# raider99k/UNINA-YOLO-DLA

Measured on NVIDIA B200. Metric: images/sec @640x640 (forward + DFL decode + NMS), higher is better.
Workload: dtype bf16

## Files before the change

unina-yolo-dla_b200/csrc/stem_fused.cu:

```cuda
#include <type_traits>

#include "camera.cuh"
#include "stem_v2.cuh"

#include "common.cuh"

namespace uyd {

struct StemArgs {
  const void *in;
  __nv_bfloat16 *out;
  const uint32_t *wfrag;
  const float *bias;
  int n, ih, iw, oh, ow, out_pitch, u8;
  int pw;
  CamFrames f;
};

namespace stemv2 {
__device__ __forceinline__ void mma1688_tf32(float (&d)[4], const uint4 &a, uint32_t b0, uint32_t b1) {
  asm volatile(
      "mma.sync.aligned.m16n8k8.row.col.f32.tf32.tf32.f32 {%0,%1,%2,%3}, {%4,%5,%6,%7}, {%8,%9}, {%0,%1,%2,%3};"
      : "+f"(d[0]), "+f"(d[1]), "+f"(d[2]), "+f"(d[3])
      : "r"(a.x), "r"(a.y), "r"(a.z), "r"(a.w), "r"(b0), "r"(b1));
}
__device__ __forceinline__ void mma16816v(float (&d)[4], const uint4 &a, uint32_t b0, uint32_t b1) {
  asm volatile(
      "mma.sync.aligned.m16n8k16.row.col.f32.bf16.bf16.f32 {%0,%1,%2,%3}, {%4,%5,%6,%7}, {%8,%9}, {%0,%1,%2,%3};"
      : "+f"(d[0]), "+f"(d[1]), "+f"(d[2]), "+f"(d[3])
      : "r"(a.x), "r"(a.y), "r"(a.z), "r"(a.w), "r"(b0), "r"(b1));
}
__device__ __forceinline__ uint32_t movmatrix_trans(uint32_t v) {
  uint32_t r;
  asm volatile("movmatrix.sync.aligned.m8n8.trans.b16 %0, %1;" : "=r"(r) : "r"(v));
  return r;
}

template <typename TIn, bool PW, bool PERSIST>
__global__ void __launch_bounds__(stemv2::kThreads, PERSIST ? 2 : 3) stem_v2_kernel(StemArgs a) {
  pdl_trigger();
  extern __shared__ __align__(16) unsigned char smem[];
  unsigned char *patch = smem;
  unsigned char *l0s = smem + kPatchBytes;
  unsigned char *w1s = smem + kPatchBytes + kL0Bytes;

  const int tid = threadIdx.x, warp = tid >> 5, lane = tid & 31, g = lane >> 2, t = lane & 3;
  uint4 w1r[PERSIST ? 18 : 1];
  if (PERSIST) {
#pragma unroll
    for (int i = 0; i < (PERSIST ? 18 : 0); ++i) w1r[i] = __ldg(reinterpret_cast<const uint4 *>(a.wfrag + kW0Words) + i * 32 + lane);
  }
  const int tiles_x = (a.ow + kTW - 1) / kTW, tiles_y = (a.oh + kTH - 1) / kTH;
  const int total_tiles = PERSIST ? tiles_x * tiles_y * a.n : 1;
  for (int tile = PERSIST ? (int)blockIdx.x : 0; tile < total_tiles; tile += PERSIST ? (int)gridDim.x : 1) {
  int ox0, oy0, n;
  if (PERSIST) {
    const int per = tiles_x * tiles_y, r = tile % per;
    n = tile / per; oy0 = (r / tiles_x) * kTH; ox0 = (r % tiles_x) * kTW;
  } else {
    ox0 = blockIdx.x * kTW; oy0 = blockIdx.y * kTH; n = blockIdx.z;
  }
  const int ix0 = 4 * ox0 - 4, iy0 = 4 * oy0 - 3;

  constexpr int kW1Vec = kW1Words / 4, kWIters = (kW1Vec + kThreads - 1) / kThreads;
  const uint4 *w1g = reinterpret_cast<const uint4 *>(a.wfrag + kW0Words);
  uint4 wv[kWIters];
#pragma unroll
  for (int it = 0; it < kWIters; ++it) {
    const int i = tid + it * kThreads;
    wv[it] = (!PERSIST && i < kW1Vec) ? __ldg(w1g + i) : make_uint4(0u, 0u, 0u, 0u);
  }
  constexpr int kVecPerRow = kInW / 4, kRowLanes = 15;
  static_assert(2 * kRowLanes <= kInH && 3 * kRowLanes >= kInH && kRowLanes * kVecPerRow <= kThreads, "patch load map");
  constexpr bool kLetterbox = std::is_same<TIn, CamLetterboxIn>::value;
  constexpr bool kCam = std::is_same<TIn, CamIn>::value || kLetterbox;
  const TIn *img = reinterpret_cast<const TIn *>(a.in) + (kCam ? 0ll : (long long)n * 3 * a.ih * a.iw);
  asm volatile("" : "+l"(img));
  const int pj = tid % kVecPerRow, prl = tid / kVecPerRow;
  const int ix = ix0 + 4 * pj;
  const bool col_ok = prl < kRowLanes && ix >= 0 && ix + 3 < a.iw;
  const unsigned plane = (unsigned)(a.ih * a.iw);
  bool ok[3];
  unsigned off[3];
#pragma unroll
  for (int k = 0; k < 3; ++k) {
    const int r = prl + kRowLanes * k, iy = iy0 + r;
    ok[k] = col_ok && r < kInH && (unsigned)iy < (unsigned)a.ih;
    off[k] = (unsigned)(iy * a.iw + ix);
  }
  uint4 pv[3][3];
  if constexpr (kCam) {
    const uint8_t *frame = reinterpret_cast<const uint8_t *>(a.in) + (long long)n * a.f.frame_stride;
    const uint8_t *uvp = a.f.uv ? a.f.uv + (long long)n * a.f.uv_frame_stride : nullptr;
    const CamNorm nm = cam_norm(a.f);
    CamLetterbox lb;
    if constexpr (kLetterbox) lb = cam_letterbox(a, a.f);
#pragma unroll
    for (int k = 0; k < 3; ++k) {
      float px[4][3];
#pragma unroll
      for (int j = 0; j < 4; ++j) px[j][0] = px[j][1] = px[j][2] = 0.f;
      if (ok[k]) {
        if constexpr (kLetterbox) cam_letterbox4(lb, a.f, nm, frame, iy0 + prl + kRowLanes * k, ix, px);
        else cam_row4(a, a.f, nm, frame, uvp, iy0 + prl + kRowLanes * k, ix, px);
      }
#pragma unroll
      for (int c = 0; c < 3; ++c)
        pv[c][k] = make_uint4(__float_as_uint(px[0][c]), __float_as_uint(px[1][c]), __float_as_uint(px[2][c]), __float_as_uint(px[3][c]));
    }
  } else {
#pragma unroll
  for (int c = 0; c < 3; ++c)
#pragma unroll
    for (int k = 0; k < 3; ++k) {
      pv[c][k] = make_uint4(0u, 0u, 0u, 0u);
      if (ok[k]) {
        const TIn *src = img + (off[k] + c * plane);
        if (sizeof(TIn) == 4) pv[c][k] = __ldg(reinterpret_cast<const uint4 *>(src));
        else pv[c][k].x = __ldg(reinterpret_cast<const unsigned int *>(src));
      }
    }
  }
#pragma unroll
  for (int it = 0; it < kWIters; ++it) {
    const int i = tid + it * kThreads;
    if (!PERSIST && i < kW1Vec) reinterpret_cast<uint4 *>(w1s)[i] = wv[it];
  }
#pragma unroll
  for (int k = 0; k < 3; ++k) {
    const int r = prl + kRowLanes * k;
    if (prl < kRowLanes && r < kInH) {
      unsigned char *dst = patch + (patch_line(0, r) * kInW + 4 * pj) * 4;
#pragma unroll
      for (int c = 0; c < 3; ++c) {
        const uint4 v = pv[c][k];
        uint4 o;
        if (sizeof(TIn) == 4 || kCam) {
          o = ok[k] ? make_uint4(v.x + 0x1000u, v.y + 0x1000u, v.z + 0x1000u, v.w + 0x1000u) : v;
        } else {
          auto cv = [&](uint32_t b) { return ok[k] ? __float_as_uint(div255((float)b)) + 0x1000u : 0u; };
          o = make_uint4(cv(v.x & 0xffu), cv((v.x >> 8) & 0xffu), cv((v.x >> 16) & 0xffu), cv(v.x >> 24));
        }
        *reinterpret_cast<uint4 *>(dst + c * kChanLines * kInW * 4) = o;
      }
    }
  }
  __syncthreads();

  {
    const uint4 *w0g = reinterpret_cast<const uint4 *>(a.wfrag);
    uint4 af[5];
#pragma unroll
    for (int s = 0; s < 5; ++s) af[s] = __ldg(w0g + s * 32 + lane);
    const float b_lo = __ldg(a.bias + g), b_hi = __ldg(a.bias + g + 8);
    const unsigned char *pb[5];
#pragma unroll
    for (int s = 0; s < 5; ++s)
      pb[s] = patch + 64 * warp + 8 * g + 8 * (t & 1) + 4 * ((t >> 1) ? l0_k_off(s, 2) : l0_k_off(s, 0));
    unsigned char *sb = l0s + (8 * warp + 2 * t) * kL0Pitch + 4 * g;
    auto groups = [&](int i0, auto cnt) {
      constexpr int NG = decltype(cnt)::value;
      float acc[NG][4];
#pragma unroll
      for (int j = 0; j < NG; ++j) { acc[j][0] = acc[j][1] = b_lo; acc[j][2] = acc[j][3] = b_hi; }
#pragma unroll
      for (int s = 0; s < 5; ++s) {
        uint2 v[NG];
#pragma unroll
        for (int j = 0; j < NG; ++j) v[j] = ld64(pb[s] + 512 * (i0 + j));
#pragma unroll
        for (int j = 0; j < NG; ++j) mma1688_tf32(acc[j], af[s], v[j].x, v[j].y);
      }
#pragma unroll
      for (int j = 0; j < NG; ++j) {
        st32(sb + 64 * kL0Pitch * (i0 + j), relu_pack_bf16(acc[j][0], acc[j][2]));
        st32(sb + 64 * kL0Pitch * (i0 + j) + kL0Pitch, relu_pack_bf16(acc[j][1], acc[j][3]));
      }
    };
    static_assert(kGroups == 73, "nine groups per warp and one more for warp 0");
    groups(0, std::integral_constant<int, 3>{});
    groups(3, std::integral_constant<int, 3>{});
    groups(6, std::integral_constant<int, 3>{});
    if (warp == 0) groups(9, std::integral_constant<int, 1>{});
  }
  __syncthreads();
  if (oy0 == 0 || ox0 == 0) {
    if (oy0 == 0)
      for (int i = tid; i < kL0P * 8; i += kThreads) st32(l0s + (i >> 3) * kL0Pitch + 4 * (i & 7), 0u);
    if (ox0 == 0 && tid < kL0H * 8) st32(l0s + (tid >> 3) * kL0P * kL0Pitch + 4 * (tid & 7), 0u);
    __syncthreads();
  }

  {
    float acc[2][2][4];
#pragma unroll
    for (int mt = 0; mt < 2; ++mt) {
      const float2 bz = __ldg(reinterpret_cast<const float2 *>(a.bias + 16 + 4 * g + 2 * mt));
#pragma unroll
      for (int xg = 0; xg < 2; ++xg) { acc[xg][mt][0] = acc[xg][mt][1] = bz.x; acc[xg][mt][2] = acc[xg][mt][3] = bz.y; }
    }
    const unsigned char *bb = l0s + l1_b_off(warp, 0, g, t, 0);
    const uint4 *wf = reinterpret_cast<const uint4 *>(w1s) + lane;
#pragma unroll
    for (int tap = 0; tap < 9; ++tap) {
      const uint4 a0 = PERSIST ? w1r[PERSIST ? tap * 2 : 0] : wf[(tap * 2 + 0) * 32], a1 = PERSIST ? w1r[PERSIST ? tap * 2 + 1 : 0] : wf[(tap * 2 + 1) * 32];
#pragma unroll
      for (int xg = 0; xg < 2; ++xg) {
        const uint2 b = ld64(bb + ((tap / 3) * kL0P + 16 * xg + tap % 3) * kL0Pitch);
        mma16816v(acc[xg][0], a0, b.x, b.y);
        mma16816v(acc[xg][1], a1, b.x, b.y);
      }
    }
    const int oy = oy0 + warp;
    __nv_bfloat16 *orow = a.out + ((long long)n * a.oh + oy) * a.ow * a.out_pitch;
    if (!PW) {
#pragma unroll
      for (int xg = 0; xg < 2; ++xg)
#pragma unroll
        for (int h = 0; h < 2; ++h) {
          const int px = ox0 + 8 * xg + 2 * t + h;
          if (oy < a.oh && px < a.ow)
            *reinterpret_cast<uint2 *>(orow + (long long)px * a.out_pitch + 4 * g) =
                make_uint2(relu_pack_bf16(acc[xg][0][h], acc[xg][0][2 + h]), relu_pack_bf16(acc[xg][1][h], acc[xg][1][2 + h]));
        }
    } else {
      const uint4 *w2 = reinterpret_cast<const uint4 *>(a.wfrag + kW0Words + kW1Words) + lane;
      const uint4 p0 = __ldg(w2), p1 = __ldg(w2 + 32);
      const float2 bz = __ldg(reinterpret_cast<const float2 *>(a.bias + 48 + 2 * g));
#pragma unroll
      for (int xg = 0; xg < 2; ++xg) {
        float acc2[4] = {bz.x, bz.x, bz.y, bz.y};
        uint32_t bq[2][2];
#pragma unroll
        for (int mt = 0; mt < 2; ++mt)
#pragma unroll
          for (int hh = 0; hh < 2; ++hh) bq[mt][hh] = movmatrix_trans(relu_pack_bf16(acc[xg][mt][2 * hh], acc[xg][mt][2 * hh + 1]));
        mma16816v(acc2, p0, bq[0][0], bq[0][1]);
        mma16816v(acc2, p1, bq[1][0], bq[1][1]);
#pragma unroll
        for (int h = 0; h < 2; ++h) {
          const int px = ox0 + 8 * xg + 2 * t + h;
          if (oy < a.oh && px < a.ow)
            *reinterpret_cast<uint32_t *>(orow + (long long)px * a.out_pitch + 2 * g) = relu_pack_bf16(acc2[h], acc2[2 + h]);
        }
      }
    }
  }
  }
}
}
bool stem_fused_supported(int c0, int c1, int ih, int iw, int out_pitch, int out_coff) {
  return c0 == 16 && c1 == 32 && ih % 4 == 0 && iw % 4 == 0 && out_pitch % 8 == 0 && out_coff % 8 == 0;
}

void stem_fused_pack(const float *w0, const float *b0, const float *w1, const float *b1, const float *w2, const float *b2,
                     std::vector<uint32_t> &frags, std::vector<float> &bias) {
  frags.clear();
  bias.assign(64, 0.f);
  for (int i = 0; i < 16; ++i) bias[i] = b0[i];
  for (int i = 0; i < 32; ++i) bias[16 + i] = b1[i];
  for (int i = 0; i < 16 && b2; ++i) bias[48 + i] = b2[i];
  stemv2::pack(w0, w1, w2, frags);
}

static int stem_v2_launch(const StemArgs &a0, cudaStream_t s) {
  StemArgs a = a0;
  static const bool persist = [] { const char *v = getenv("UYD_STEM_PERSIST"); return !(v && *v == '0'); }();
  const int sms = current_sm_count();
  UYD_REQUIRE(sms > 0, UYD_E_NOGPU, "stem: no current CUDA device");
  const int tiles = ceil_div(a.ow, stemv2::kTW) * ceil_div(a.oh, stemv2::kTH) * a.n;
  const size_t smem = stemv2::kSmemBytes;
  auto go = [&](auto kern, bool pers) -> int {
    if (int e = smem_optin(kern, stemv2::kSmemBytes)) return e;
    if (pers) kern<<<tiles < 2 * sms ? tiles : 2 * sms, stemv2::kThreads, smem, s>>>(a);
    else kern<<<dim3(ceil_div(a.ow, stemv2::kTW), ceil_div(a.oh, stemv2::kTH), a.n), stemv2::kThreads, smem, s>>>(a);
    return (int)cudaGetLastError();
  };
  const bool pers = persist && tiles >= 8 * sms;
  using namespace stemv2;
  if (a.f.cam == UYD_CAM_BGRA_LETTERBOX) {
    if (a.pw) return pers ? go(stem_v2_kernel<CamLetterboxIn, true, true>, true) : go(stem_v2_kernel<CamLetterboxIn, true, false>, false);
    return pers ? go(stem_v2_kernel<CamLetterboxIn, false, true>, true) : go(stem_v2_kernel<CamLetterboxIn, false, false>, false);
  }
  if (a.f.cam) {
    if (a.pw) return pers ? go(stem_v2_kernel<CamIn, true, true>, true) : go(stem_v2_kernel<CamIn, true, false>, false);
    return pers ? go(stem_v2_kernel<CamIn, false, true>, true) : go(stem_v2_kernel<CamIn, false, false>, false);
  }
  if (a.u8) {
    if (a.pw) return pers ? go(stem_v2_kernel<uint8_t, true, true>, true) : go(stem_v2_kernel<uint8_t, true, false>, false);
    return pers ? go(stem_v2_kernel<uint8_t, false, true>, true) : go(stem_v2_kernel<uint8_t, false, false>, false);
  }
  if (a.pw) return pers ? go(stem_v2_kernel<float, true, true>, true) : go(stem_v2_kernel<float, true, false>, false);
  return pers ? go(stem_v2_kernel<float, false, true>, true) : go(stem_v2_kernel<float, false, false>, false);
}

int stem_fused_launch(const StemArgs &a, cudaStream_t s) { return stem_v2_launch(a, s); }

}
```

unina-yolo-dla_b200/csrc/stem_v2.cuh:

```cuda
#pragma once
#include "c3k_flat.cuh"

namespace uyd {
namespace stemv2 {
using c3kf::host_f2bf;
using c3kf::ld64;
using c3kf::relu_pack_bf16;
using c3kf::st32;

constexpr int kTH = 8, kTW = 16;
constexpr int kL0H = 2 * kTH + 1, kL0P = 2 * kTW + 2;
constexpr int kGroups = (16 * kL0P + 2 * kTW + 1 + 7) / 8;
constexpr int kL0Px = kGroups * 8;
constexpr int kInH = 2 * kL0H + 1, kInW = 2 * kL0P;
constexpr int kOddLine = 20, kChanLines = 38;
constexpr int kL0Pitch = 48;
constexpr int kPatchBytes = 3 * kChanLines * kInW * 4;
constexpr int kL0Bytes = kL0Px * kL0Pitch;
constexpr int kW0Words = 5 * 128, kW1Words = 9 * 2 * 128, kW2Words = 2 * 128;
constexpr int kSmemBytes = kPatchBytes + kL0Bytes + kW1Words * 4;
constexpr int kThreads = 256;
constexpr int kFragWords = kW0Words + kW1Words + kW2Words;

C3K_HD int patch_line(int c, int r) { return c * kChanLines + ((r & 1) ? kOddLine + (r >> 1) : (r >> 1)); }

C3K_HD int l0_k_off(int s, int t) {
  int c = 2 * s + (t >> 1);
  if (c > 8) c = 8;
  const int ky = c % 3;
  return (patch_line(c / 3, ky & 1) + (ky >> 1)) * kInW + 2 * (t & 1);
}
inline float l0_weight(const float *w0, int s, int k, int n) {
  const int t = k & 3, combo = 2 * s + (t >> 1), slot = 2 * (t & 1) + (k >> 2), kx = slot - 1;
  if (combo > 8 || kx < 0) return 0.f;
  return w0[((n * 3 + combo / 3) * 3 + combo % 3) * 3 + kx];
}
C3K_HD void l0_store(unsigned char *l0s, int q, int g, float lo_ch, float hi_ch) { st32(l0s + q * kL0Pitch + 4 * g, relu_pack_bf16(lo_ch, hi_ch)); }

C3K_HD int l1_k_chan(int kk) { return 2 * ((kk & 7) >> 1) + (kk >> 3) + 8 * (kk & 1); }
C3K_HD int l1_b_off(int row, int xg, int g, int t, int tap) {
  return ((2 * row + tap / 3) * kL0P + 2 * (8 * xg + g) + tap % 3) * kL0Pitch + 8 * t;
}
C3K_HD int l1_chan(int mt, int r) { return 4 * (r & 7) + 2 * mt + (r >> 3); }

C3K_HD int pw_chan(int r) { return 2 * (r & 7) + (r >> 3); }

inline uint32_t f32_bits(float f) { uint32_t u; memcpy(&u, &f, 4); return u; }
inline float bits_f32(uint32_t u) { float f; memcpy(&f, &u, 4); return f; }
inline float bf16_round(float f) { return bits_f32((uint32_t)host_f2bf(f) << 16); }

C3K_HD float div255(float x) {
#if defined(__CUDA_ARCH__)
  const float r = 1.0f / 255.0f;
  const float q = __fmul_rn(x, r);
  return __fmaf_rn(__fmaf_rn(-q, 255.0f, x), r, q);
#else
  return x / 255.0f;
#endif
}

inline void pack(const float *w0, const float *w1, const float *w2 , std::vector<uint32_t> &out) {
  for (int s = 0; s < 5; ++s)
    for (int lane = 0; lane < 32; ++lane) {
      const int g = lane >> 2, t = lane & 3;
      auto w = [&](int row, int k) { return f32_bits(bf16_round(l0_weight(w0, s, k, row))); };
      out.push_back(w(g, t)); out.push_back(w(g + 8, t)); out.push_back(w(g, t + 4)); out.push_back(w(g + 8, t + 4));
    }
  for (int tap = 0; tap < 9; ++tap)
    for (int mt = 0; mt < 2; ++mt)
      for (int lane = 0; lane < 32; ++lane) {
        const int g = lane >> 2, t = lane & 3;
        auto w = [&](int row, int kk) {
          auto one = [&](int k1) { return (uint32_t)host_f2bf(w1[(l1_chan(mt, row) * 16 + l1_k_chan(k1)) * 9 + tap]); };
          return one(kk) | (one(kk + 1) << 16);
        };
        out.push_back(w(g, 2 * t)); out.push_back(w(g + 8, 2 * t)); out.push_back(w(g, 2 * t + 8)); out.push_back(w(g + 8, 2 * t + 8));
      }
  for (int ks = 0; ks < 2; ++ks)
    for (int lane = 0; lane < 32; ++lane) {
      const int g = lane >> 2, t = lane & 3;
      auto w = [&](int row, int kk) {
        auto one = [&](int k1) { return w2 ? (uint32_t)host_f2bf(w2[pw_chan(row) * 32 + l1_chan(ks, k1)]) : 0u; };
        return one(kk) | (one(kk + 1) << 16);
      };
      out.push_back(w(g, 2 * t)); out.push_back(w(g + 8, 2 * t)); out.push_back(w(g, 2 * t + 8)); out.push_back(w(g + 8, 2 * t + 8));
    }
}

}
}
```

Before: 32890.

## Load fp32 stem input patches with double-buffered TMA in persistent kernel

Adds a TMA path for fp32 non-camera input in the persistent stem kernel. A 4D tensor map splits even and odd rows, and thread 0 prefetches the next tile's 3-channel patch into a second shared-memory buffer, tracked by mbarriers. This replaces per-thread global loads and shared stores. Out-of-bounds zero fill replaces the explicit edge masking, and the tf32 rounding offset is now applied at fragment load time. The cost is a larger shared-memory footprint and a host-side tensor map encode on every launch.

```diff
diff --git a/unina-yolo-dla_b200/csrc/stem_fused.cu b/unina-yolo-dla_b200/csrc/stem_fused.cu
--- a/unina-yolo-dla_b200/csrc/stem_fused.cu
+++ b/unina-yolo-dla_b200/csrc/stem_fused.cu
@@ -4,6 +4,7 @@
 #include "stem_v2.cuh"
 
 #include "common.cuh"
+#include "tc_ptx.cuh"
 
 namespace uyd {
 
@@ -36,13 +37,31 @@
   return r;
 }
 
+struct TmaF32 {};
+template <typename TIn>
+using StemMap = typename std::conditional<std::is_same<TIn, TmaF32>::value, CUtensorMap, char>::type;
+
+__device__ __forceinline__ void stem_tma_patch(const CUtensorMap *tm, unsigned char *buf, uint32_t bar, int ox0, int oy0, int n) {
+  mbar_expect_tx(bar, 6 * kTmaRows * kInW * 4);
+#pragma unroll
+  for (int c = 0; c < 3; ++c)
+#pragma unroll
+    for (int odd = 0; odd < 2; ++odd) {
+      const int line0 = patch_line(c, odd, true), lead = tma_lead(c, odd);
+      tma_load_4d(smem_u32(buf + (line0 - lead) * kInW * 4), tm, bar, 4 * ox0 - 4, 1 - odd, 2 * oy0 - 2 + odd - lead, 3 * n + c);
+    }
+}
+
 template <typename TIn, bool PW, bool PERSIST>
-__global__ void __launch_bounds__(stemv2::kThreads, PERSIST ? 2 : 3) stem_v2_kernel(StemArgs a) {
+__global__ void __launch_bounds__(stemv2::kThreads, PERSIST ? 2 : 3) stem_v2_kernel(StemArgs a, const __grid_constant__ StemMap<TIn> tm) {
+  constexpr bool kTma = std::is_same<TIn, TmaF32>::value;
+  static_assert(!kTma || PERSIST, "the TMA patch pipeline walks tiles");
   pdl_trigger();
-  extern __shared__ __align__(16) unsigned char smem[];
+  extern __shared__ __align__(128) unsigned char smem[];
   unsigned char *patch = smem;
-  unsigned char *l0s = smem + kPatchBytes;
+  unsigned char *l0s = smem + (kTma ? 2 * kTmaBufBytes : kPatchBytes);
   unsigned char *w1s = smem + kPatchBytes + kL0Bytes;
+  const uint32_t full_bar = smem_u32(smem + 2 * kTmaBufBytes + kL0Bytes);
 
   const int tid = threadIdx.x, warp = tid >> 5, lane = tid & 31, g = lane >> 2, t = lane & 3;
   uint4 w1r[PERSIST ? 18 : 1];
@@ -52,6 +71,22 @@
   }
   const int tiles_x = (a.ow + kTW - 1) / kTW, tiles_y = (a.oh + kTH - 1) / kTH;
   const int total_tiles = PERSIST ? tiles_x * tiles_y * a.n : 1;
+  auto tile_origin = [&](int tile, int &ox0, int &oy0, int &n) {
+    const int per = tiles_x * tiles_y, r = tile % per;
+    n = tile / per; oy0 = (r / tiles_x) * kTH; ox0 = (r % tiles_x) * kTW;
+  };
+  if constexpr (kTma) {
+    if (tid == 0) {
+      mbar_init(full_bar, 1);
+      mbar_init(full_bar + 8, 1);
+      fence_barrier_init();
+      int ox0, oy0, n;
+      tile_origin(blockIdx.x, ox0, oy0, n);
+      stem_tma_patch(&tm, smem, full_bar, ox0, oy0, n);
+    }
+    __syncthreads();
+  }
+  int iter = 0;
   for (int tile = PERSIST ? (int)blockIdx.x : 0; tile < total_tiles; tile += PERSIST ? (int)gridDim.x : 1) {
   int ox0, oy0, n;
   if (PERSIST) {
@@ -60,6 +95,17 @@
   } else {
     ox0 = blockIdx.x * kTW; oy0 = blockIdx.y * kTH; n = blockIdx.z;
   }
+  if constexpr (kTma) {
+    const int next = tile + (int)gridDim.x;
+    if (tid == 0 && next < total_tiles) {
+      int nx0, ny0, nn;
+      tile_origin(next, nx0, ny0, nn);
+      stem_tma_patch(&tm, smem + ((iter + 1) & 1) * kTmaBufBytes, full_bar + 8 * ((iter + 1) & 1), nx0, ny0, nn);
+    }
+    patch = smem + (iter & 1) * kTmaBufBytes;
+    mbar_wait(full_bar + 8 * (iter & 1), (iter >> 1) & 1);
+    ++iter;
+  } else {
   const int ix0 = 4 * ox0 - 4, iy0 = 4 * oy0 - 3;
 
   constexpr int kW1Vec = kW1Words / 4, kWIters = (kW1Vec + kThreads - 1) / kThreads;
@@ -145,6 +191,7 @@
       }
     }
   }
+  }
   __syncthreads();
 
   {
@@ -156,7 +203,7 @@
     const unsigned char *pb[5];
 #pragma unroll
     for (int s = 0; s < 5; ++s)
-      pb[s] = patch + 64 * warp + 8 * g + 8 * (t & 1) + 4 * ((t >> 1) ? l0_k_off(s, 2) : l0_k_off(s, 0));
+      pb[s] = patch + 64 * warp + 8 * g + 8 * (t & 1) + 4 * ((t >> 1) ? l0_k_off(s, 2, kTma) : l0_k_off(s, 0, kTma));
     unsigned char *sb = l0s + (8 * warp + 2 * t) * kL0Pitch + 4 * g;
     auto groups = [&](int i0, auto cnt) {
       constexpr int NG = decltype(cnt)::value;
@@ -167,7 +214,10 @@
       for (int s = 0; s < 5; ++s) {
         uint2 v[NG];
 #pragma unroll
-        for (int j = 0; j < NG; ++j) v[j] = ld64(pb[s] + 512 * (i0 + j));
+        for (int j = 0; j < NG; ++j) {
+          v[j] = ld64(pb[s] + 512 * (i0 + j));
+          if (kTma) { v[j].x += 0x1000u; v[j].y += 0x1000u; }
+        }
 #pragma unroll
         for (int j = 0; j < NG; ++j) mma1688_tf32(acc[j], af[s], v[j].x, v[j].y);
       }
@@ -263,21 +313,56 @@
   stemv2::pack(w0, w1, w2, frags);
 }
 
+typedef CUresult (*EncodeTiledFn)(CUtensorMap *, CUtensorMapDataType, cuuint32_t, void *, const cuuint64_t *, const cuuint64_t *,
+                                  const cuuint32_t *, const cuuint32_t *, CUtensorMapInterleave, CUtensorMapSwizzle,
+                                  CUtensorMapL2promotion, CUtensorMapFloatOOBfill);
+
+static int stem_frame_map(const StemArgs &a, CUtensorMap *tm) {
+  static EncodeTiledFn fn = [] {
+    void *q = nullptr;
+    cudaDriverEntryPointQueryResult r;
+    return cudaGetDriverEntryPoint("cuTensorMapEncodeTiled", &q, cudaEnableDefault, &r) == cudaSuccess && r == cudaDriverEntryPointSuccess
+               ? reinterpret_cast<EncodeTiledFn>(q) : nullptr;
+  }();
+  UYD_REQUIRE(fn, UYD_E_NOGPU, "cuTensorMapEncodeTiled is not available (no CUDA driver)");
+  const cuuint64_t w = (cuuint64_t)a.iw, h = (cuuint64_t)a.ih;
+  const cuuint64_t dims[4] = {w, 2, h / 2, 3 * (cuuint64_t)a.n};
+  const cuuint64_t str[3] = {w * 4, 2 * w * 4, h * w * 4};
+  const cuuint32_t box[4] = {(cuuint32_t)stemv2::kInW, 1, (cuuint32_t)stemv2::kTmaRows, 1};
+  const cuuint32_t one[4] = {1, 1, 1, 1};
+  CUresult r = fn(tm, CU_TENSOR_MAP_DATA_TYPE_FLOAT32, 4, const_cast<void *>(a.in), dims, str, box, one, CU_TENSOR_MAP_INTERLEAVE_NONE,
+                  CU_TENSOR_MAP_SWIZZLE_NONE, CU_TENSOR_MAP_L2_PROMOTION_L2_128B, CU_TENSOR_MAP_FLOAT_OOB_FILL_NONE);
+  UYD_REQUIRE(r == CUDA_SUCCESS, UYD_E_ARG, "stem: cuTensorMapEncodeTiled failed with CUresult %d", (int)r);
+  return UYD_OK;
+}
+
 static int stem_v2_launch(const StemArgs &a0, cudaStream_t s) {
   StemArgs a = a0;
   static const bool persist = [] { const char *v = getenv("UYD_STEM_PERSIST"); return !(v && *v == '0'); }();
+  const char *tma_env = getenv("UYD_STEM_TMA");
+  const bool tma = !(tma_env && *tma_env == '0');
   const int sms = current_sm_count();
   UYD_REQUIRE(sms > 0, UYD_E_NOGPU, "stem: no current CUDA device");
   const int tiles = ceil_div(a.ow, stemv2::kTW) * ceil_div(a.oh, stemv2::kTH) * a.n;
-  const size_t smem = stemv2::kSmemBytes;
+  const int grid_pers = tiles < 2 * sms ? tiles : 2 * sms;
   auto go = [&](auto kern, bool pers) -> int {
-    if (int e = smem_optin(kern, stemv2::kSmemBytes)) return e;
-    if (pers) kern<<<tiles < 2 * sms ? tiles : 2 * sms, stemv2::kThreads, smem, s>>>(a);
-    else kern<<<dim3(ceil_div(a.ow, stemv2::kTW), ceil_div(a.oh, stemv2::kTH), a.n), stemv2::kThreads, smem, s>>>(a);
+    const size_t smem = stemv2::kSmemBytes;
+    if (int e = smem_optin(kern, smem)) return e;
+    if (pers) kern<<<grid_pers, stemv2::kThreads, smem, s>>>(a, 0);
+    else kern<<<dim3(ceil_div(a.ow, stemv2::kTW), ceil_div(a.oh, stemv2::kTH), a.n), stemv2::kThreads, smem, s>>>(a, 0);
     return (int)cudaGetLastError();
   };
   const bool pers = persist && tiles >= 8 * sms;
   using namespace stemv2;
+  if (pers && tma && !a.u8 && !a.f.cam) {
+    UYD_REQUIRE((reinterpret_cast<uintptr_t>(a.in) & 15) == 0, UYD_E_UNSUPPORTED, "stem: fp32 frames must be 16-byte aligned");
+    CUtensorMap tm;
+    if (int e = stem_frame_map(a, &tm)) return e;
+    auto kern = a.pw ? stem_v2_kernel<TmaF32, true, true> : stem_v2_kernel<TmaF32, false, true>;
+    if (int e = smem_optin(kern, kTmaSmemBytes)) return e;
+    kern<<<grid_pers, kThreads, kTmaSmemBytes, s>>>(a, tm);
+    return (int)cudaGetLastError();
+  }
   if (a.f.cam == UYD_CAM_BGRA_LETTERBOX) {
     if (a.pw) return pers ? go(stem_v2_kernel<CamLetterboxIn, true, true>, true) : go(stem_v2_kernel<CamLetterboxIn, true, false>, false);
     return pers ? go(stem_v2_kernel<CamLetterboxIn, false, true>, true) : go(stem_v2_kernel<CamLetterboxIn, false, false>, false);
diff --git a/unina-yolo-dla_b200/csrc/stem_v2.cuh b/unina-yolo-dla_b200/csrc/stem_v2.cuh
--- a/unina-yolo-dla_b200/csrc/stem_v2.cuh
+++ b/unina-yolo-dla_b200/csrc/stem_v2.cuh
@@ -22,13 +22,21 @@
 constexpr int kThreads = 256;
 constexpr int kFragWords = kW0Words + kW1Words + kW2Words;
 
-C3K_HD int patch_line(int c, int r) { return c * kChanLines + ((r & 1) ? kOddLine + (r >> 1) : (r >> 1)); }
+constexpr int kTmaRows = 21, kTmaRegionLines = 24;
+constexpr int kTmaBufBytes = 6 * kTmaRegionLines * kInW * 4;
+constexpr int kTmaSmemBytes = 2 * kTmaBufBytes + kL0Bytes + 16;
+C3K_HD int tma_lead(int c, int odd) { return odd ? (c == 1 ? 4 : c == 2 ? 3 : 0) : (c == 0 ? 3 : 0); }
 
-C3K_HD int l0_k_off(int s, int t) {
+C3K_HD int patch_line(int c, int r, bool tma = false) {
+  if (tma) return (2 * c + (r & 1)) * kTmaRegionLines + tma_lead(c, r & 1) + (r >> 1);
+  return c * kChanLines + ((r & 1) ? kOddLine + (r >> 1) : (r >> 1));
+}
+
+C3K_HD int l0_k_off(int s, int t, bool tma = false) {
   int c = 2 * s + (t >> 1);
   if (c > 8) c = 8;
   const int ky = c % 3;
-  return (patch_line(c / 3, ky & 1) + (ky >> 1)) * kInW + 2 * (t & 1);
+  return (patch_line(c / 3, ky & 1, tma) + (ky >> 1)) * kInW + 2 * (t & 1);
 }
 inline float l0_weight(const float *w0, int s, int k, int n) {
   const int t = k & 3, combo = 2 * s + (t >> 1), slot = 2 * (t & 1) + (k >> 2), kx = slot - 1;
```

Result: faster. 33610, median of 6 (+2.2%).
